# 2thleZ/flash_attention_metal

Hardware: AMD Instinct MI355X
Metric: attn_fwd_tflops (seqlen=4096, head_dim=64, bf16, causal) (higher is better)
Workload: dtype bf16; 1 GPU; BASELINE.json configs[2]: seqlen=4096 head_dim=64 batch=4 heads=16 bf16 is_causal=true per GPU; batch_per_gpu=4, heads=16, seq_len=4096, head_dim=64, is_causal=True

## Files before the change

### flash_attention_metal_amd/csrc/fa_mfma16_kernel.hip

```cpp
#include <stdlib.h>

#include <algorithm>

#include "fa_mfma_common.h"

#ifndef FA16_DEFER_THR
#define FA16_DEFER_THR 8.0f
#endif
#ifndef FA16_LAK
#define FA16_LAK (D == 128 ? 3 : 2)
#endif
#ifndef FA16_LAV
#define FA16_LAV (D == 128 ? 3 : 2)
#endif
#ifndef FA16_PRIO
#define FA16_PRIO 1
#endif
#ifndef FA16_ONES
#define FA16_ONES 1
#endif
#ifndef FA16_HALVES
#define FA16_HALVES 0
#endif
#ifndef FA16_BN128
#define FA16_BN128 64
#endif
#ifndef FA16_OCC128
#define FA16_OCC128 2
#endif
#ifndef FA16_SUB8
#define FA16_SUB8 1
#endif
#ifndef FA16_OCC
#define FA16_OCC 4
#endif

namespace fa {

typedef float f32x4 __attribute__((ext_vector_type(4)));

template <typename Tag> struct MT16;
template <> struct MT16<BF16> {
  using elem = __bf16;
  using vec8 = bf16x8;
  __device__ static __forceinline__ f32x4 mfma(vec8 a, vec8 b, f32x4 c) { return __builtin_amdgcn_mfma_f32_16x16x32_bf16(a, b, c, 0, 0, 0); }
};
template <> struct MT16<F16> {
  using elem = _Float16;
  using vec8 = f16x8;
  __device__ static __forceinline__ f32x4 mfma(vec8 a, vec8 b, f32x4 c) { return __builtin_amdgcn_mfma_f32_16x16x32_f16(a, b, c, 0, 0, 0); }
};

__device__ __forceinline__ float xlane(float x, int mask) { return __shfl_xor(x, mask, 64); }

template <typename Tag, int D, bool CAUSAL, int RW, bool PAD, int SUB>
__device__ __forceinline__ void fwd_mfma16_body(const Params &p) {
  using M = MT16<Tag>;
  using vec8 = typename M::vec8;
  using elem = typename M::elem;
  constexpr int BMR = RW * WM;
  constexpr int RB = D * 2;
  constexpr int CPR = D / 8;
  constexpr int KS = D / 32;
  constexpr int DT = D / 16;
  constexpr int BNK = (D == 128) ? FA16_BN128 : BN;
  constexpr int KT = BNK / 16;
  constexpr int NKP = KT / 2;
  constexpr int TILE = BNK * RB;
  static_assert(D == 64 || D == 128, "head dims of the 16x16x32 kernel");

  extern __shared__ __attribute__((aligned(16))) char smem_generic[];
  lds_char *smem = (lds_char *)smem_generic;
  lds_char *Kbuf = smem;
  lds_char *Vbuf = smem + 2 * SUB * TILE;

  const int wave = __builtin_amdgcn_readfirstlane((int)threadIdx.x >> 6);
  const int lane = threadIdx.x & 63;
  const int c = lane & 15;
  const int g = lane >> 4;

  int bh, qb;
  map_block<CAUSAL>(blockIdx.x, p, bh, qb);
  long long base, base_kv;
  head_bases(bh, p, base, base_kv);
  const int coff = p.Nk - p.N;
  const int q0 = qb * BMR;
  const int qw0 = q0 + wave * WM;

  const int GRB = PAD ? p.D * 2 : RB;
  auto gcol = [&](int chunk) -> unsigned { return (!PAD || chunk * 8 < p.D) ? (unsigned)chunk * 16 : 0x80000000u; };
  const unsigned head_bytes = (unsigned)p.N * GRB, kv_head_bytes = (unsigned)p.Nk * GRB;
  const __amdgpu_buffer_rsrc_t rq = __builtin_amdgcn_make_buffer_rsrc((void *)((const char *)p.q + base * 2), 0, head_bytes, 0x00020000);
  const __amdgpu_buffer_rsrc_t rk = __builtin_amdgcn_make_buffer_rsrc((void *)((const char *)p.k + base_kv * 2), 0, kv_head_bytes, 0x00020000);
  const __amdgpu_buffer_rsrc_t rv = __builtin_amdgcn_make_buffer_rsrc((void *)((const char *)p.v + base_kv * 2), 0, kv_head_bytes, 0x00020000);

  vec8 qf[2][KS];
#pragma unroll
  for (int qt = 0; qt < 2; ++qt)
#pragma unroll
    for (int ks = 0; ks < KS; ++ks) {
      const u32x4 t = __builtin_amdgcn_raw_buffer_load_b128(rq, (unsigned)(qw0 + 16 * qt + c) * GRB + gcol(4 * ks + g), 0, 0);
      qf[qt][ks] = __builtin_bit_cast(vec8, t);
    }

  const int kx = (D == 64) ? ((c >> 1) & 7) : c;
  const lds_char *kptr[KS];
#pragma unroll
  for (int ks = 0; ks < KS; ++ks) {
    kptr[ks] = Kbuf + c * RB + (((4 * ks + g) ^ kx) << 4);
    asm volatile("" : "+v"(kptr[ks]));
  }
  const int vq = c >> 2, vp = c & 3;
  const int vrow = 4 * g + vq;
  const int vx = (D == 64) ? (((vrow >> 1) & 3) << 1) : ((vrow & 7) << 1);
  const lds_char *vptr[DT];
#pragma unroll
  for (int dt = 0; dt < DT; ++dt) {
    vptr[dt] = Vbuf + vrow * RB + ((((2 * dt) ^ vx) + (vp >> 1)) << 4) + 8 * (vp & 1);
    asm volatile("" : "+v"(vptr[dt]));
  }

  const int kv_end = CAUSAL ? min(p.Nk, q0 + BMR + coff) : p.Nk;
  const int nT = (kv_end + BNK - 1) / BNK;

  constexpr int RPP = 1024 / RB;
  constexpr int NPW = (BNK / RPP) / RW;
  static_assert((RW * RPP) % 16 == 0, "the piece stride must keep the swizzle");
  unsigned dma_kvo, dma_vvo;
  {
    const int row = wave * RPP + lane / CPR, pc = lane % CPR;
    const int skx = (D == 64) ? ((row >> 1) & 7) : (row & 15);
    const int svx = (D == 64) ? (((row >> 1) & 3) << 1) : ((row & 7) << 1);
    dma_kvo = (unsigned)(row * GRB) + gcol(pc ^ skx);
    dma_vvo = (unsigned)(row * GRB) + gcol(pc ^ svx);
  }
  auto stage_dma = [&](int t, int buf) {
#pragma unroll
    for (int j = 0; j < NPW; ++j) {
      const unsigned soff = PAD ? (unsigned)(t * BNK + j * RW * RPP) * GRB : (unsigned)t * TILE + j * (RW * 1024);
      const unsigned lk = (unsigned)(__UINTPTR_TYPE__)Kbuf + buf * TILE + (wave + RW * j) * 1024;
      const unsigned lv = (unsigned)(__UINTPTR_TYPE__)Vbuf + buf * TILE + (wave + RW * j) * 1024;
      asm volatile("s_mov_b32 m0, %0\n\ts_nop 0\n\tbuffer_load_dwordx4 %1, %2, %3 offen lds" ::"s"(lk), "v"(dma_kvo), "s"(rk), "s"(soff) : "memory");
      asm volatile("s_mov_b32 m0, %0\n\ts_nop 0\n\tbuffer_load_dwordx4 %1, %2, %3 offen lds" ::"s"(lv), "v"(dma_vvo), "s"(rv), "s"(soff) : "memory");
    }
  };

  f32x4 oacc[DT][2];
#pragma unroll
  for (int dt = 0; dt < DT; ++dt)
#pragma unroll
    for (int qt = 0; qt < 2; ++qt)
#pragma unroll
      for (int i = 0; i < 4; ++i) oacc[dt][qt][i] = 0.0f;
  constexpr bool ONES = (FA16_ONES != 0);
  constexpr float BIAS = !ONES ? 0.0f : std::is_same<Tag, F16>::value ? 3.0f : 7.0f;
  constexpr float FIRST_SUM_FLOOR = std::is_same<Tag, F16>::value ? 1.0f : 0x1p-64f;
  float l[2] = {0.0f, 0.0f};
  f32x4 lacc[2];
#pragma unroll
  for (int qt = 0; qt < 2; ++qt)
#pragma unroll
    for (int i = 0; i < 4; ++i) lacc[qt][i] = 0.0f;
  vec8 ones;
#pragma unroll
  for (int j = 0; j < 8; ++j) ones[j] = (elem)1.0f;
  if constexpr (ONES) asm volatile("" : "+v"(ones));
  const float c2 = p.scale * 1.4426950408889634f;
  f32x4 negm[2];
#pragma unroll
  for (int qt = 0; qt < 2; ++qt) {
#pragma unroll
    for (int i = 0; i < 4; ++i) negm[qt][i] = ONES ? -BIAS : INFINITY;
    asm volatile("" : "+v"(negm[qt]));
  }

  stage_dma(0, 0);
  if constexpr (SUB == 2) {
    if (1 < nT) stage_dma(1, 1);
  }
  asm volatile("s_waitcnt vmcnt(0)" ::: "memory");
#pragma unroll
  for (int qt = 0; qt < 2; ++qt)
#pragma unroll
    for (int ks = 0; ks < KS; ++ks) {
#pragma unroll
      for (int j = 0; j < 8; ++j) qf[qt][ks][j] = (elem)((float)qf[qt][ks][j] * c2);
      asm volatile("" : "+v"(qf[qt][ks]));
    }
  __syncthreads();

  const float sum_thr = __builtin_exp2f(FA16_DEFER_THR);
  auto apply_mask = [&](auto k0c, auto &s, const int kv0) __attribute__((always_inline)) {
    constexpr int K0 = decltype(k0c)::value;
    constexpr int NKT = sizeof(s) / sizeof(s[0]);
    int g4 = 4 * g;
    asm volatile("" : "+v"(g4));
#pragma unroll
    for (int qt = 0; qt < 2; ++qt) {
      int lim = p.Nk - 1 - kv0 - g4;
      if (CAUSAL) lim = min(lim, qw0 + 16 * qt + c + coff - kv0 - g4);
#pragma unroll
      for (int k2 = 0; k2 < NKT; ++k2)
#pragma unroll
        for (int i = 0; i < 4; ++i) s[k2][qt][i] = (16 * (K0 + k2) + i > lim) ? -INFINITY : s[k2][qt][i];
    }
  };
  auto needs_mask = [&](const int kv0) __attribute__((always_inline)) { return (CAUSAL && (kv0 + BNK - 1 > qw0 + coff)) || (kv0 + BNK > p.Nk); };
  auto score_group = [&](auto bufc, auto k0c, auto &s, const f32x4 c0, const f32x4 c1) __attribute__((always_inline)) {
    constexpr int buf = decltype(bufc)::value;
    constexpr int K0 = decltype(k0c)::value;
    constexpr int NKT = sizeof(s) / sizeof(s[0]);
    constexpr int NK = NKT * KS, LA = (FA16_LAK < NK) ? FA16_LAK : NK;
    vec8 kf[NK];
    auto kread = [&](int i) { kf[i] = __builtin_bit_cast(vec8, lds_read_b128(kptr[i % KS] + buf * TILE + (K0 + i / KS) * 16 * RB)); };
#pragma unroll
    for (int i = 0; i < LA; ++i) kread(i);
    __builtin_amdgcn_sched_barrier(0);
#pragma unroll
    for (int i = 0; i < NK; ++i) {
      const int k2 = i / KS, ks = i % KS;
      s[k2][0] = M::mfma(kf[i], qf[0][ks], ks == 0 ? c0 : s[k2][0]);
      s[k2][1] = M::mfma(kf[i], qf[1][ks], ks == 0 ? c1 : s[k2][1]);
      if (i + LA < NK) kread(i + LA);
      __builtin_amdgcn_sched_barrier(0);
    }
  };
  auto pack_group = [&](auto k0c, auto &s, vec8 (&pf)[NKP][2], unsigned &bits) __attribute__((always_inline)) {
    constexpr int K0 = decltype(k0c)::value;
    constexpr int NKT = sizeof(s) / sizeof(s[0]);
#pragma unroll
    for (int kp = 0; kp < NKT / 2; ++kp)
#pragma unroll
      for (int qt = 0; qt < 2; ++qt) {
#pragma unroll
        for (int j = 0; j < 8; ++j) pf[K0 / 2 + kp][qt][j] = (elem)s[2 * kp + (j >> 2)][qt][j & 3];
        if constexpr (ONES) {
          const u32x4 w = __builtin_bit_cast(u32x4, pf[K0 / 2 + kp][qt]);
          bits |= w[0] | w[1] | w[2] | w[3];
        }
      }
  };
  auto hot_group = [&](auto bufc, auto k0c, auto nktc, const int kv0, vec8 (&pf)[NKP][2], unsigned &bits,
                       float (&ls)[2]) __attribute__((always_inline)) {
    constexpr int NKT = decltype(nktc)::value;
    f32x4 s[NKT][2];
    score_group(bufc, k0c, s, negm[0], negm[1]);
    if (needs_mask(kv0)) apply_mask(k0c, s, kv0);
#if FA16_PRIO
    if constexpr (decltype(k0c)::value + NKT == KT) __builtin_amdgcn_s_setprio(0);
#endif
#pragma unroll
    for (int k2 = 0; k2 < NKT; ++k2)
#pragma unroll
      for (int i = 0; i < 4; ++i)
#pragma unroll
        for (int qt = 0; qt < 2; ++qt) {
          s[k2][qt][i] = __builtin_amdgcn_exp2f(s[k2][qt][i]);
          if constexpr (!ONES) ls[qt] = (decltype(k0c)::value == 0 && k2 == 0 && i == 0) ? s[k2][qt][i] : ls[qt] + s[k2][qt][i];
        }
    pack_group(k0c, s, pf, bits);
  };
  auto max_group = [&](auto bufc, auto k0c, auto nktc, const int kv0, float (&mx)[2]) __attribute__((always_inline)) {
    constexpr int NKT = decltype(nktc)::value;
    f32x4 s[NKT][2], zero;
#pragma unroll
    for (int i = 0; i < 4; ++i) zero[i] = 0.0f;
    score_group(bufc, k0c, s, zero, zero);
    if (needs_mask(kv0)) apply_mask(k0c, s, kv0);
#pragma unroll
    for (int qt = 0; qt < 2; ++qt)
#pragma unroll
      for (int k2 = 0; k2 < NKT; ++k2)
#pragma unroll
        for (int i = 0; i < 4; ++i) mx[qt] = fmaxf(mx[qt], s[k2][qt][i]);
  };
  auto new_reference = [&](auto firstc, float (&mx)[2]) __attribute__((always_inline)) {
    constexpr bool FIRST = decltype(firstc)::value;
#pragma unroll
    for (int qt = 0; qt < 2; ++qt) {
      float v = mx[qt];
      v = fmaxf(v, xlane(v, 16));
      v = fmaxf(v, xlane(v, 32));
      const float m_old = -negm[qt][0];
      const float m_new = FIRST ? v + BIAS : fmaxf(m_old, v + BIAS);
#pragma unroll
      for (int i = 0; i < 4; ++i) negm[qt][i] = -m_new;
      asm volatile("" : "+v"(negm[qt]));
      if constexpr (FIRST) continue;
      const float alpha = __builtin_amdgcn_exp2f(m_old - m_new);
      if constexpr (ONES) {
#pragma unroll
        for (int i = 0; i < 4; ++i) lacc[qt][i] *= alpha;
      } else {
        l[qt] *= alpha;
      }
#pragma unroll
      for (int dt = 0; dt < DT; ++dt)
#pragma unroll
        for (int i = 0; i < 4; ++i) oacc[dt][qt][i] *= alpha;
    }
  };
  constexpr int G = (FA16_HALVES != 0) ? 2 : 1;
  using KTG = std::integral_constant<int, KT / G>;
  using K0A = std::integral_constant<int, 0>;
  using K0B = std::integral_constant<int, KT / 2>;

  auto tile = [&](auto bufc, auto firstc, const int t) {
    constexpr int buf = decltype(bufc)::value;
    constexpr bool FIRST = decltype(firstc)::value;
    const int kv0 = t * BNK;

    int always = 1;
    if constexpr (!CAUSAL) asm volatile("" : "+s"(always));
    const bool wave_active = CAUSAL ? (kv0 <= qw0 + WM - 1 + coff) : (always != 0);
    if (wave_active) {
      vec8 pf[NKP][2];
      float ls[2] = {0.0f, 0.0f};
      bool redo = FIRST && !ONES;
      for (;;) {
        if (__builtin_expect(redo, 0)) {
          float mx[2] = {-INFINITY, -INFINITY};
          max_group(bufc, K0A{}, std::integral_constant<int, KT / 2>{}, kv0, mx);
          max_group(bufc, K0B{}, std::integral_constant<int, KT / 2>{}, kv0, mx);
          new_reference(firstc, mx);
        }
#if FA16_PRIO
        __builtin_amdgcn_s_setprio(1);
#endif
        unsigned bits = 0;
        hot_group(bufc, K0A{}, KTG{}, kv0, pf, bits, ls);
        if constexpr (G == 2) hot_group(bufc, K0B{}, KTG{}, kv0, pf, bits, ls);
        bool stale;
        if constexpr (ONES) stale = __builtin_amdgcn_ballot_w64((bits & 0x40004000u) != 0) != 0;
        else stale = __builtin_amdgcn_ballot_w64(fmaxf(ls[0], ls[1]) > sum_thr) != 0;
        if (__builtin_expect(stale && !redo, 0)) {
          redo = true;
          continue;
        }
        if constexpr (!ONES) {
          l[0] += ls[0];
          l[1] += ls[1];
        }
#if FA16_PRIO
        __builtin_amdgcn_s_setprio(1);
#endif
        {
          constexpr int NV = NKP * DT, LA = FA16_LAV;
          s16x4 wlo[NV], whi[NV];
          auto vread = [&](int j) {
            const lds_char *vb = vptr[j % DT] + buf * TILE + (32 * (j / DT)) * RB;
            wlo[j] = lds_read_tr16(vb);
            whi[j] = lds_read_tr16(vb + 16 * RB);
          };
#pragma unroll
          for (int j = 0; j < LA; ++j) vread(j);
          __builtin_amdgcn_sched_barrier(0);
#pragma unroll
          for (int j = 0; j < NV; ++j) {
            const s16x8 v8 = __builtin_shufflevector(wlo[j], whi[j], 0, 1, 2, 3, 4, 5, 6, 7);
#pragma unroll
            for (int qt = 0; qt < 2; ++qt) oacc[j % DT][qt] = M::mfma(__builtin_bit_cast(vec8, v8), pf[j / DT][qt], oacc[j % DT][qt]);
            if (j + LA < NV) vread(j + LA);
            if constexpr (ONES) {
              if (j % DT == DT - 1) {
#pragma unroll
                for (int qt = 0; qt < 2; ++qt) lacc[qt] = M::mfma(ones, pf[j / DT][qt], lacc[qt]);
              }
            }
            __builtin_amdgcn_sched_barrier(0);
          }
        }
#if FA16_PRIO
        __builtin_amdgcn_s_setprio(0);
#endif
        if constexpr (FIRST && ONES) {
          if (__builtin_expect(!redo && __builtin_amdgcn_ballot_w64(fminf(lacc[0][0], lacc[1][0]) < FIRST_SUM_FLOOR) != 0, 0)) {
#pragma unroll
            for (int qt = 0; qt < 2; ++qt) {
#pragma unroll
              for (int i = 0; i < 4; ++i) lacc[qt][i] = 0.0f;
#pragma unroll
              for (int dt = 0; dt < DT; ++dt)
#pragma unroll
                for (int i = 0; i < 4; ++i) oacc[dt][qt][i] = 0.0f;
            }
            redo = true;
            continue;
          }
        }
        break;
      }
    }
  };
  auto unit = [&](auto bufc, auto firstc, const int t0) {
    constexpr int buf = decltype(bufc)::value;
#pragma unroll
    for (int sub = 0; sub < SUB; ++sub)
      if (t0 + SUB + sub < nT) stage_dma(t0 + SUB + sub, (buf ^ 1) * SUB + sub);
    tile(std::integral_constant<int, buf * SUB>{}, firstc, t0);
    if constexpr (SUB == 2) {
      if (t0 + 1 < nT) tile(std::integral_constant<int, buf * SUB + 1>{}, std::false_type{}, t0 + 1);
    }
    if (t0 + SUB < nT) asm volatile("s_waitcnt vmcnt(0)" ::: "memory");
    __syncthreads();
  };
  unit(std::integral_constant<int, 0>{}, std::true_type{}, 0);
  for (int t = SUB; t < nT; t += 2 * SUB) {
    unit(std::integral_constant<int, 1>{}, std::false_type{}, t);
    if (t + SUB < nT) unit(std::integral_constant<int, 0>{}, std::false_type{}, t + SUB);
  }

  lds_char *Ot = smem + wave * (WM * RB);
#pragma unroll
  for (int qt = 0; qt < 2; ++qt) {
    float lt = ONES ? lacc[qt][0] : l[qt];
    if constexpr (!ONES) {
      lt += xlane(lt, 16);
      lt += xlane(lt, 32);
    }
    const float inv_l = __builtin_amdgcn_rcpf(lt);
    const int row = 16 * qt + c, qrow = qw0 + row;
    if (p.lse != nullptr && g == 0 && qrow < p.N)
      p.lse[(long long)bh * p.N + qrow] = (__builtin_amdgcn_logf(lt) - negm[qt][0]) * 0.6931471805599453f;
#pragma unroll
    for (int dt = 0; dt < DT; ++dt) {
      typedef elem elem4 __attribute__((ext_vector_type(4)));
      elem4 e;
#pragma unroll
      for (int i = 0; i < 4; ++i) e[i] = (elem)(oacc[dt][qt][i] * inv_l);
      const u32x2 w = __builtin_bit_cast(u32x2, e);
      const int ch = (2 * dt + (g >> 1)) ^ (row & (CPR - 1));
      lds_write_b64(Ot + row * RB + (ch << 4) + 8 * (g & 1), w);
    }
  }
  __syncthreads();
  {
    elem *Og = (elem *)p.o + base;
#pragma unroll
    for (int it = 0; it < WM * CPR / 64; ++it) {
      const int idx = it * 64 + lane;
      const int row = idx / CPR, ch = idx % CPR;
      const u32x4 vv = lds_read_b128(Ot + row * RB + ((ch ^ (row & (CPR - 1))) << 4));
      if (qw0 + row < p.N && (!PAD || ch * 8 < p.D)) *reinterpret_cast<u32x4 *>(Og + (long long)(qw0 + row) * (PAD ? p.D : D) + ch * 8) = vv;
    }
  }
}

template <typename Tag, int D, bool CAUSAL, int RW, bool PAD = false, int SUB = 1>
__global__ __launch_bounds__(64 * RW, (D == 64 ? FA16_OCC : FA16_OCC128)) void fwd_mfma16_kernel(Params p) {
  fwd_mfma16_body<Tag, D, CAUSAL, RW, PAD, SUB>(p);
}

bool mfma16_supported(int dtype, int D) { return (dtype == FA_DTYPE_F16 || dtype == FA_DTYPE_BF16) && D >= 8 && D <= 128 && D % 8 == 0; }

template <typename Tag, int D, bool CAUSAL, int RW, bool PAD = false, int SUB = 1>
static hipError_t launch16_one(const Params &p, hipStream_t s) {
  const int nQ = (p.N + RW * WM - 1) / (RW * WM);
  const size_t smem = 4 * SUB * (size_t)(D == 128 ? FA16_BN128 : BN) * D * 2;
  auto kern = fwd_mfma16_kernel<Tag, D, CAUSAL, RW, PAD, SUB>;
  if (smem > 48 * 1024) {
    hipError_t e = set_dyn_lds_once((const void *)kern, (int)smem);
    if (e != hipSuccess) return e;
  }
  Params pp = p;
  pp.head_group = causal_head_group(p, D, 2);
#ifdef FA16_FORCE_HEAD_GROUP
  pp.head_group = FA16_FORCE_HEAD_GROUP;
#endif
  set_block_divisors(pp, nQ, pp.head_group);
  (void)hipGetLastError();
  hipLaunchKernelGGL(kern, dim3(nQ * p.B * p.H), dim3(64 * RW), smem, s, pp);
  return hipGetLastError();
}

int mfma16_waves(int D, int BH, int N, int Nk, int is_causal) {
#ifdef FA16_FORCE_RW
  return FA16_FORCE_RW;
#endif
  if (D != 64 && D != 128) return 4;
  const long long b256 = (long long)BH * ((N + 255) / 256);
  if (D == 128) return (!is_causal && Nk >= 8192 && b256 >= 1024) ? 8 : 4;
  if (!is_causal) return (Nk >= 512 && b256 >= 512) ? 8 : 4;
  return (Nk >= 4096 && Nk < 6144 && b256 >= 1024 && b256 < 1280) ? 8 : 4;
}

hipError_t launch_mfma16(const Params &p, int dtype, hipStream_t s) {
  const bool w8 = mfma16_waves(p.D, p.B * p.H, p.N, p.Nk, p.is_causal) == 8 && (p.D == 64 || !p.is_causal);
  auto go = [&](auto tag) -> hipError_t {
    using Tag = decltype(tag);
    if (p.D != 64 && p.D != 128) {
      if (p.D < 64) return p.is_causal ? launch16_one<Tag, 64, true, 4, true>(p, s) : launch16_one<Tag, 64, false, 4, true>(p, s);
      return p.is_causal ? launch16_one<Tag, 128, true, 4, true>(p, s) : launch16_one<Tag, 128, false, 4, true>(p, s);
    }
    if (p.D == 64) {
      if (w8) return p.is_causal ? launch16_one<Tag, 64, true, 8, false, FA16_SUB8>(p, s) : launch16_one<Tag, 64, false, 8, false, FA16_SUB8>(p, s);
      return p.is_causal ? launch16_one<Tag, 64, true, 4>(p, s) : launch16_one<Tag, 64, false, 4>(p, s);
    }
    if (p.D == 128) {
      if (w8) return launch16_one<Tag, 128, false, 8>(p, s);
      return p.is_causal ? launch16_one<Tag, 128, true, 4>(p, s) : launch16_one<Tag, 128, false, 4>(p, s);
    }
    return hipErrorInvalidValue;
  };
  return dtype == FA_DTYPE_F16 ? go(F16{}) : go(BF16{});
}

}
```

Measured before the change: 1128 TFLOP/s.

## Replace per-tile stale-max ballot with lazy exponent renormalisation for bf16 D=64

After: 1146 TFLOP/s, median of 6. +1.6%, better.

```diff
diff --git a/flash_attention_metal_amd/csrc/fa_mfma16_kernel.hip b/flash_attention_metal_amd/csrc/fa_mfma16_kernel.hip
--- a/flash_attention_metal_amd/csrc/fa_mfma16_kernel.hip
+++ b/flash_attention_metal_amd/csrc/fa_mfma16_kernel.hip
@@ -18,6 +18,15 @@
 #endif
 #ifndef FA16_ONES
 #define FA16_ONES 1
+#endif
+#ifndef FA16_LAZY
+#define FA16_LAZY 1
+#endif
+#ifndef FA16_LAZY_THR
+#define FA16_LAZY_THR 0x1p20f
+#endif
+#ifndef FA16_LAZY_POISON
+#define FA16_LAZY_POISON 0x1p64f
 #endif
 #ifndef FA16_HALVES
 #define FA16_HALVES 0
@@ -153,6 +162,10 @@
 #pragma unroll
       for (int i = 0; i < 4; ++i) oacc[dt][qt][i] = 0.0f;
   constexpr bool ONES = (FA16_ONES != 0);
+  constexpr bool LAZY = ONES && std::is_same<Tag, BF16>::value && D == 64 && (FA16_LAZY != 0);
+  constexpr bool LAZY_TEST = LAZY && (FA16_LAZY == 1);
+  lds_char *poison_flag = smem + 4 * SUB * TILE;
+  int slow = 0;
   constexpr float BIAS = !ONES ? 0.0f : std::is_same<Tag, F16>::value ? 3.0f : 7.0f;
   constexpr float FIRST_SUM_FLOOR = std::is_same<Tag, F16>::value ? 1.0f : 0x1p-64f;
   float l[2] = {0.0f, 0.0f};
@@ -174,6 +187,9 @@
     asm volatile("" : "+v"(negm[qt]));
   }
 
+  if constexpr (LAZY_TEST) {
+    if (threadIdx.x == 0) lds_write_b32(poison_flag, 0u);
+  }
   stage_dma(0, 0);
   if constexpr (SUB == 2) {
     if (1 < nT) stage_dma(1, 1);
@@ -234,17 +250,20 @@
       for (int qt = 0; qt < 2; ++qt) {
 #pragma unroll
         for (int j = 0; j < 8; ++j) pf[K0 / 2 + kp][qt][j] = (elem)s[2 * kp + (j >> 2)][qt][j & 3];
-        if constexpr (ONES) {
+        if constexpr (ONES && !LAZY) {
           const u32x4 w = __builtin_bit_cast(u32x4, pf[K0 / 2 + kp][qt]);
           bits |= w[0] | w[1] | w[2] | w[3];
         }
       }
   };
-  auto hot_group = [&](auto bufc, auto k0c, auto nktc, const int kv0, vec8 (&pf)[NKP][2], unsigned &bits,
-                       float (&ls)[2]) __attribute__((always_inline)) {
+  auto hot_group = [&](auto bufc, auto k0c, auto nktc, const int kv0, vec8 (&pf)[NKP][2], unsigned &bits, float (&ls)[2],
+                       const bool leave) __attribute__((always_inline)) -> bool {
     constexpr int NKT = decltype(nktc)::value;
     f32x4 s[NKT][2];
     score_group(bufc, k0c, s, negm[0], negm[1]);
+    if constexpr (LAZY_TEST) {
+      if (__builtin_expect(leave, 0)) return true;
+    }
     if (needs_mask(kv0)) apply_mask(k0c, s, kv0);
 #if FA16_PRIO
     if constexpr (decltype(k0c)::value + NKT == KT) __builtin_amdgcn_s_setprio(0);
@@ -259,6 +278,7 @@
           if constexpr (!ONES) ls[qt] = (decltype(k0c)::value == 0 && k2 == 0 && i == 0) ? s[k2][qt][i] : ls[qt] + s[k2][qt][i];
         }
     pack_group(k0c, s, pf, bits);
+    return false;
   };
   auto max_group = [&](auto bufc, auto k0c, auto nktc, const int kv0, float (&mx)[2]) __attribute__((always_inline)) {
     constexpr int NKT = decltype(nktc)::value;
@@ -300,6 +320,34 @@
         for (int i = 0; i < 4; ++i) oacc[dt][qt][i] *= alpha;
     }
   };
+  constexpr unsigned LAZY_THR_BITS = __builtin_bit_cast(unsigned, (float)FA16_LAZY_THR);
+  constexpr unsigned LAZY_POISON_BITS = __builtin_bit_cast(unsigned, (float)FA16_LAZY_POISON);
+  static_assert(LAZY_THR_BITS < LAZY_POISON_BITS && LAZY_POISON_BITS < 0x7f800000u, "2^-BIAS << THR < POISON < inf");
+  auto lazy_renormalise = [&]() __attribute__((always_inline)) {
+    const unsigned b0 = __builtin_bit_cast(unsigned, lacc[0][0]), b1 = __builtin_bit_cast(unsigned, lacc[1][0]);
+    if (__builtin_expect(__builtin_amdgcn_ballot_w64(max(b0, b1) >= LAZY_THR_BITS) != 0, 0)) {
+#pragma unroll
+      for (int qt = 0; qt < 2; ++qt) {
+        const unsigned a = __builtin_bit_cast(unsigned, lacc[qt][0]) & 0x7fffffffu;
+        const bool bad = a >= LAZY_POISON_BITS;
+        const bool big = !bad && a >= LAZY_THR_BITS;
+        const int e = (int)(a >> 23) - 127;
+        const float sc = big ? __builtin_bit_cast(float, (unsigned)(127 - e) << 23) : 1.0f;
+        const float kf = big ? (float)e : 0.0f;
+#pragma unroll
+        for (int i = 0; i < 4; ++i) {
+          lacc[qt][i] *= sc;
+          negm[qt][i] -= kf;
+        }
+        asm volatile("" : "+v"(negm[qt]));
+#pragma unroll
+        for (int dt = 0; dt < DT; ++dt)
+#pragma unroll
+          for (int i = 0; i < 4; ++i) oacc[dt][qt][i] *= sc;
+        if (bad) lds_write_b32(poison_flag, 1u);
+      }
+    }
+  };
   constexpr int G = (FA16_HALVES != 0) ? 2 : 1;
   using KTG = std::integral_constant<int, KT / G>;
   using K0A = std::integral_constant<int, 0>;
@@ -316,6 +364,7 @@
     if (wave_active) {
       vec8 pf[NKP][2];
       float ls[2] = {0.0f, 0.0f};
+      if constexpr (LAZY_TEST && !FIRST) lazy_renormalise();
       bool redo = FIRST && !ONES;
       for (;;) {
         if (__builtin_expect(redo, 0)) {
@@ -328,10 +377,18 @@
         __builtin_amdgcn_s_setprio(1);
 #endif
         unsigned bits = 0;
-        hot_group(bufc, K0A{}, KTG{}, kv0, pf, bits, ls);
-        if constexpr (G == 2) hot_group(bufc, K0B{}, KTG{}, kv0, pf, bits, ls);
+        if constexpr (LAZY_TEST) {
+          if (hot_group(bufc, K0A{}, KTG{}, kv0, pf, bits, ls, slow != 0 && !redo)) {
+            redo = true;
+            continue;
+          }
+        } else {
+          hot_group(bufc, K0A{}, KTG{}, kv0, pf, bits, ls, false);
+        }
+        if constexpr (G == 2) hot_group(bufc, K0B{}, KTG{}, kv0, pf, bits, ls, false);
         bool stale;
-        if constexpr (ONES) stale = __builtin_amdgcn_ballot_w64((bits & 0x40004000u) != 0) != 0;
+        if constexpr (LAZY) stale = false;
+        else if constexpr (ONES) stale = __builtin_amdgcn_ballot_w64((bits & 0x40004000u) != 0) != 0;
         else stale = __builtin_amdgcn_ballot_w64(fmaxf(ls[0], ls[1]) > sum_thr) != 0;
         if (__builtin_expect(stale && !redo, 0)) {
           redo = true;
@@ -402,14 +459,54 @@
       if (t0 + 1 < nT) tile(std::integral_constant<int, buf * SUB + 1>{}, std::false_type{}, t0 + 1);
     }
     if (t0 + SUB < nT) asm volatile("s_waitcnt vmcnt(0)" ::: "memory");
+    if constexpr (LAZY_TEST) {
+      if (t0 + SUB >= nT && slow == 0) {
+        const unsigned a0 = __builtin_bit_cast(unsigned, lacc[0][0]) & 0x7fffffffu, a1 = __builtin_bit_cast(unsigned, lacc[1][0]) & 0x7fffffffu;
+        if (max(a0, a1) >= LAZY_POISON_BITS) lds_write_b32(poison_flag, 1u);
+      }
+    }
     __syncthreads();
   };
-  unit(std::integral_constant<int, 0>{}, std::true_type{}, 0);
-  for (int t = SUB; t < nT; t += 2 * SUB) {
-    unit(std::integral_constant<int, 1>{}, std::false_type{}, t);
-    if (t + SUB < nT) unit(std::integral_constant<int, 0>{}, std::false_type{}, t + SUB);
-  }
-
+  for (;;) {
+    unit(std::integral_constant<int, 0>{}, std::true_type{}, 0);
+    for (int t = SUB; t < nT; t += 2 * SUB) {
+      unit(std::integral_constant<int, 1>{}, std::false_type{}, t);
+      if (t + SUB < nT) unit(std::integral_constant<int, 0>{}, std::false_type{}, t + SUB);
+    }
+    if constexpr (LAZY_TEST) {
+      if (slow == 0) {
+        const unsigned f = *reinterpret_cast<const volatile __attribute__((address_space(3))) unsigned *>(poison_flag);
+        if (__builtin_expect(__builtin_amdgcn_readfirstlane((int)f) != 0, 0)) {
+          slow = 1;
+#pragma unroll
+          for (int qt = 0; qt < 2; ++qt) {
+#pragma unroll
+            for (int i = 0; i < 4; ++i) {
+              lacc[qt][i] = 0.0f;
+              negm[qt][i] = -BIAS;
+            }
+            asm volatile("" : "+v"(negm[qt]));
+#pragma unroll
+            for (int dt = 0; dt < DT; ++dt)
+#pragma unroll
+              for (int i = 0; i < 4; ++i) oacc[dt][qt][i] = 0.0f;
+          }
+          stage_dma(0, 0);
+          if constexpr (SUB == 2) {
+            if (1 < nT) stage_dma(1, 1);
+          }
+          asm volatile("s_waitcnt vmcnt(0)" ::: "memory");
+          __syncthreads();
+          continue;
+        }
+      }
+    }
+    break;
+  }
+
+  int elane = lane;
+  if constexpr (LAZY_TEST) asm volatile("" : "+v"(elane));
+  const int ec = elane & 15, eg = elane >> 4;
   lds_char *Ot = smem + wave * (WM * RB);
 #pragma unroll
   for (int qt = 0; qt < 2; ++qt) {
@@ -419,8 +516,8 @@
       lt += xlane(lt, 32);
     }
     const float inv_l = __builtin_amdgcn_rcpf(lt);
-    const int row = 16 * qt + c, qrow = qw0 + row;
-    if (p.lse != nullptr && g == 0 && qrow < p.N)
+    const int row = 16 * qt + ec, qrow = qw0 + row;
+    if (p.lse != nullptr && eg == 0 && qrow < p.N)
       p.lse[(long long)bh * p.N + qrow] = (__builtin_amdgcn_logf(lt) - negm[qt][0]) * 0.6931471805599453f;
 #pragma unroll
     for (int dt = 0; dt < DT; ++dt) {
@@ -429,8 +526,8 @@
 #pragma unroll
       for (int i = 0; i < 4; ++i) e[i] = (elem)(oacc[dt][qt][i] * inv_l);
       const u32x2 w = __builtin_bit_cast(u32x2, e);
-      const int ch = (2 * dt + (g >> 1)) ^ (row & (CPR - 1));
-      lds_write_b64(Ot + row * RB + (ch << 4) + 8 * (g & 1), w);
+      const int ch = (2 * dt + (eg >> 1)) ^ (row & (CPR - 1));
+      lds_write_b64(Ot + row * RB + (ch << 4) + 8 * (eg & 1), w);
     }
   }
   __syncthreads();
@@ -438,7 +535,7 @@
     elem *Og = (elem *)p.o + base;
 #pragma unroll
     for (int it = 0; it < WM * CPR / 64; ++it) {
-      const int idx = it * 64 + lane;
+      const int idx = it * 64 + elane;
       const int row = idx / CPR, ch = idx % CPR;
       const u32x4 vv = lds_read_b128(Ot + row * RB + ((ch ^ (row & (CPR - 1))) << 4));
       if (qw0 + row < p.N && (!PAD || ch * 8 < p.D)) *reinterpret_cast<u32x4 *>(Og + (long long)(qw0 + row) * (PAD ? p.D : D) + ch * 8) = vv;
@@ -456,7 +553,8 @@
 template <typename Tag, int D, bool CAUSAL, int RW, bool PAD = false, int SUB = 1>
 static hipError_t launch16_one(const Params &p, hipStream_t s) {
   const int nQ = (p.N + RW * WM - 1) / (RW * WM);
-  const size_t smem = 4 * SUB * (size_t)(D == 128 ? FA16_BN128 : BN) * D * 2;
+  constexpr bool lazy = std::is_same<Tag, BF16>::value && D == 64 && (FA16_ONES != 0) && (FA16_LAZY == 1);
+  const size_t smem = 4 * SUB * (size_t)(D == 128 ? FA16_BN128 : BN) * D * 2 + (lazy ? 16 : 0);
   auto kern = fwd_mfma16_kernel<Tag, D, CAUSAL, RW, PAD, SUB>;
   if (smem > 48 * 1024) {
     hipError_t e = set_dyn_lds_once((const void *)kern, (int)smem);
```
